# wendongbi/Bridged-GNN

Hardware: AMD Instinct MI355X
Metric: aggregated_edges_per_sec_ktgnn_fwd (higher is better)
Workload: dtype f32; 1 GPU; C4 synthetic bridged graph (local) N=1000000 E'=20991058, 2-layer KT-GNN eval fwd F=128 hidden=128 C=2; parallelism=single, execution=eager launches

## Files before the change

### bridged_gnn_amd/csrc/bgnn_aggregate.hip

```cpp
#include <cstdlib>
#include "bgnn_common.h"

namespace {

struct AggParams {
  const float* h_t2s;
  const float* h_s2t;
  int64_t ldh;
  const float* a_t2s;
  const float* a_s2t;
  const int32_t* rowptr;
  const int32_t* col;
  const uint8_t* mask;
  int64_t row_begin;
  int64_t row_end;
  int32_t D;
  float slope;
  float* out;
  int64_t ldo;
  float* alpha;
  const float* ep_scale;
  const float* ep_shift;
  int ep_relu;
  unsigned int* tile_queue;
// ... 857 lines not shown
  (void)ntiles; (void)grid;
  return forced > 0 ? forced : 4;
}

template <int HEADS, int EP, int U>
int launch_heads(const AggParams& p, hipStream_t st) {
  constexpr int RPB = 4 * (64 / (EP * HEADS));
  static const int cap = [] {
    int per_cu = 0, dev = 0;
    hipDeviceProp_t prop;
    if (hipGetDevice(&dev) != hipSuccess || hipGetDeviceProperties(&prop, dev) != hipSuccess) return 2048;
    if (hipOccupancyMaxActiveBlocksPerMultiprocessor(&per_cu, agg_heads_lanes_kernel<HEADS, EP, U>, 256, 0) != hipSuccess || per_cu < 1) return 2048;
    if (per_cu > 8) per_cu = 8;
    return per_cu * prop.multiProcessorCount / 8 * 8;
  }();
  const int64_t ntiles = (p.row_end - p.row_begin + p.n_vrows + RPB - 1) / RPB;
  int64_t grid = ntiles < cap ? (ntiles + 7) / 8 * 8 : cap;
  if (grid < 8) grid = 8;
  hipLaunchKernelGGL((agg_heads_lanes_kernel<HEADS, EP, U>), dim3((unsigned)grid), dim3(256), 0, st, p);
  BGNN_LAUNCH_CHECK();
  return 0;
}

template <int LF, int EP, int U>
int resident_blocks() {
  static const int nb = [] {
    int per_cu = 0, dev = 0;
    hipDeviceProp_t prop;
    if (hipGetDevice(&dev) != hipSuccess || hipGetDeviceProperties(&prop, dev) != hipSuccess) return 2048;
    if (hipOccupancyMaxActiveBlocksPerMultiprocessor(&per_cu, agg_kernel<LF, EP, U>, 256, 0) != hipSuccess || per_cu < 1)
      return 2048;
    if (per_cu > 8) per_cu = 8;
    return per_cu * prop.multiProcessorCount / 8 * 8;
  }();
  return nb;
}

template <int LF, int EP, int U>
int launch(const AggParams& p, hipStream_t st) {
  constexpr int RPB = 4 * (64 / (LF * EP));
  int64_t ntiles = ((p.row_end - p.row_begin) * p.heads + RPB - 1) / RPB;
  const int64_t cap = resident_blocks<LF, EP, U>();
  int64_t grid = ntiles < cap ? (ntiles + 7) / 8 * 8 : cap;
  if (grid < 8) grid = 8;
  AggParams q = p;
  q.tq_chunk = tq_chunk_for(ntiles, grid);
// ... 27 lines not shown
  hipLaunchKernelGGL((agg_wide_kernel<LF, U>), dim3((unsigned)grid), dim3(256), 0, st, q);
  BGNN_LAUNCH_CHECK();
  return 0;
}

static bool fast_plan(AggParams& p, int64_t table_rows) {
  static const bool on = [] { const char* e = getenv("BGNN_AGG_FAST"); return !(e && atoi(e) == 0); }();
  if (!on || table_rows <= 0) return false;
  if (p.heads != 1 || p.mode != 0 || p.n_vrows != 0 || p.hub_threshold != 0) return false;
  const int64_t lim24 = (int64_t)1 << 24, lim32 = ((int64_t)1 << 32) - 1;
  if (table_rows > lim24 || p.row_end > table_rows || p.ldh * 4 >= lim24 || p.ldo * 4 >= lim24) return false;
  const char* a = reinterpret_cast<const char*>(p.h_t2s);
  const char* b = reinterpret_cast<const char*>(p.h_s2t);
  const char* lo = a < b ? a : b;
  const int64_t span = (int64_t)((a < b ? b : a) - lo) + table_rows * p.ldh * 4;
  if (span > lim32 || p.row_end * p.ldo * 4 > lim32) return false;
  p.tbl_base = lo;
  p.tbl_bytes = (uint32_t)span;
  p.off_t2s = (uint32_t)(a - lo);
  p.off_s2t = (uint32_t)(b - lo);
  const int64_t lane_max = (span - table_rows * p.ldh * 4) + p.ldh * 4, dead = (((int64_t)1 << 32) - 16) - lane_max;
  p.dead_off = dead >= span ? (uint32_t)dead : 0u;
  return true;
}

template <int LF, bool ALPHA>
int launch_wide_fast(const AggParams& p, hipStream_t st) {
  constexpr int RPB = 4 * (64 / LF);
  static const int per_cu_max = [] {
    int per_cu = 0;
    if (hipOccupancyMaxActiveBlocksPerMultiprocessor(&per_cu, agg_wide_fast_kernel<LF, ALPHA>, 256, 0) != hipSuccess || per_cu < 1) return 0;
    if (per_cu > 8) per_cu = 8;
    const char* e = getenv("BGNN_AGG_BLOCKS_PER_CU");
    if (e && atoi(e) > 0 && atoi(e) < per_cu) per_cu = atoi(e);
    return per_cu;
  }();
  static const int n_cu = [] {
    int dev = 0;
    hipDeviceProp_t prop;
    if (hipGetDevice(&dev) != hipSuccess || hipGetDeviceProperties(&prop, dev) != hipSuccess) return 0;
    return prop.multiProcessorCount;
  }();
  static const bool forced = getenv("BGNN_AGG_BLOCKS_PER_CU") != nullptr;
  int per_cu = per_cu_max;
  if (p.gather_hint == 2 && !forced && per_cu > 3) per_cu = 3;
  const int64_t cap = (per_cu_max > 0 && n_cu > 0) ? (int64_t)per_cu * n_cu / 8 * 8 : 2048;
// ... 125 lines not shown
    p.state_ms[2 * (node * p.heads + h)] = m;
    p.state_ms[2 * (node * p.heads + h) + 1] = s;
  }
  if (p.ep_relu == 2) {
    float mx = r.x;
    if (p.D > 1) mx = fmaxf(mx, r.y);
    if (p.D > 2) mx = fmaxf(mx, r.z);
    if (p.D > 3) mx = fmaxf(mx, r.w);
    float se = expf(r.x - mx);
    if (p.D > 1) se += expf(r.y - mx);
    if (p.D > 2) se += expf(r.z - mx);
    if (p.D > 3) se += expf(r.w - mx);
    const float lse = logf(se);
    r.x = r.x - mx - lse;
    r.y = p.D > 1 ? r.y - mx - lse : 0.f;
    r.z = p.D > 2 ? r.z - mx - lse : 0.f;
    r.w = p.D > 3 ? r.w - mx - lse : 0.f;
  }
  *reinterpret_cast<float4*>(p.out + (node * p.heads + h) * p.ldo) = r;
}

static int dispatch_aggregate(const AggParams& p, hipStream_t st, int64_t table_rows = 0) {
  const int32_t D = p.D, heads = p.heads;
  if (heads == 3 && D <= 4 && p.ldh == 4 && p.ldo == 4) return launch_heads<3, 2, 4>(p, st);
  if (heads == 2 && D <= 4 && p.ldh == 4 && p.ldo == 4) return launch_heads<2, 2, 4>(p, st);
  const int nv = (D + 3) / 4;
  if (nv <= 1) return launch<1, 4, 4>(p, st);
  if (nv <= 2) return launch<2, 2, 4>(p, st);
  if (nv <= 4) return launch<4, 1, 8>(p, st);
  if (nv <= 8) return launch<8, 1, 4>(p, st);
  const bool wide_ok = p.slope >= 0.f && p.slope <= 1.f && (int64_t)heads * p.ldh * 4 < (int64_t)1 << 32;
  if (wide_ok) {
    AggParams q = p;
    if (fast_plan(q, table_rows)) {
      if (q.alpha != nullptr) {
        if (nv <= 16) return launch_wide_fast<16, true>(q, st);
        if (nv <= 32) return launch_wide_fast<32, true>(q, st);
        return launch_wide_fast<64, true>(q, st);
      }
      if (nv <= 16) return launch_wide_fast<16, false>(q, st);
      if (nv <= 32) return launch_wide_fast<32, false>(q, st);
      return launch_wide_fast<64, false>(q, st);
    }
    if (nv <= 16) return launch_wide<16, 4>(p, st);
    if (nv <= 32) return launch_wide<32, 4>(p, st);
    return launch_wide<64, 4>(p, st);
  }
// ... 14 lines not shown
                          const float* a_t2s, const float* a_s2t,
                          const int32_t* rowptr, const int32_t* col, const uint8_t* mask,
                          int64_t row_begin, int64_t row_end, int32_t D, float negative_slope,
                          float* out, int64_t ldo, float* alpha_opt,
                          const float* ep_scale_opt, const float* ep_shift_opt, int ep_relu,
                          float* state_ms_opt, int part, int64_t park_begin, int32_t heads,
                          double* colsum_opt, uint32_t* tile_queue_opt, int64_t table_rows, int32_t gather_hint, void* stream) {
  if (colsum_opt && heads != 1) return BGNN_E_SHAPE;
  if (part == 1 && (park_begin < row_begin || park_begin > row_end)) return BGNN_E_SHAPE;
  if (part < 0 || part > 3 || (part != 0 && (!state_ms_opt || alpha_opt))) return BGNN_E_NULL;
  if (part == 3 && !((heads == 3 || heads == 2) && D <= 4 && ldh == 4 && ldo == 4)) return BGNN_E_SHAPE;
  if (heads < 1 || heads > 8 || (heads > 1 && (alpha_opt || ep_scale_opt))) return BGNN_E_SHAPE;
  if (ep_relu < 0 || ep_relu > 2) return BGNN_E_SHAPE;
  if (ep_relu == 2 && !((heads == 3 || heads == 2) && D <= 4 && ldh == 4 && ldo == 4)) return BGNN_E_SHAPE;
  if (!h_t2s || !h_s2t || !a_t2s || !a_s2t || !rowptr || !col || !mask || !out) return BGNN_E_NULL;
  if (row_begin < 0 || row_end < row_begin || D <= 0 || D > 256 || ldh < D || ldo < D) return BGNN_E_SHAPE;
  if ((ldh & 3) || (ldo & 3) || !bgnn_aligned16(h_t2s) || !bgnn_aligned16(h_s2t) || !bgnn_aligned16(out))
    return BGNN_E_ALIGN;
  if ((ep_scale_opt == nullptr) != (ep_shift_opt == nullptr)) return BGNN_E_NULL;
  if (row_end == row_begin) return 0;
  AggParams p{h_t2s, h_s2t, ldh, a_t2s, a_s2t, rowptr, col, mask, row_begin, row_end, D, negative_slope,
              out, ldo, alpha_opt, ep_scale_opt, ep_shift_opt, ep_relu, tile_queue_opt, colsum_opt, heads, state_ms_opt, part,
              park_begin, 4};
  p.gather_hint = gather_hint;
  hipStream_t st = (hipStream_t)stream;
  if (tile_queue_opt) {
    hipError_t e = bgnn_zero_async(tile_queue_opt, 8 * sizeof(uint32_t), st);
    if (e != hipSuccess) return (int)e;
  }
  return dispatch_aggregate(p, st, table_rows);
}

extern "C" int bgnn_adaptedconv_aggregate_f32(const float* h_t2s, const float* h_s2t, int64_t ldh,
                                              const float* a_t2s, const float* a_s2t,
                                              const int32_t* rowptr, const int32_t* col, const uint8_t* mask,
                                              int64_t row_begin, int64_t row_end, int32_t D, float negative_slope,
                                              float* out, int64_t ldo, float* alpha_opt,
                                              const float* ep_scale_opt, const float* ep_shift_opt, int ep_relu,
                                              float* state_ms_opt, int part, int64_t park_begin, int32_t heads,
                                              double* colsum_opt, uint32_t* tile_queue_opt, void* stream) {
  return aggregate_impl(h_t2s, h_s2t, ldh, a_t2s, a_s2t, rowptr, col, mask, row_begin, row_end, D, negative_slope, out, ldo, alpha_opt,
                        ep_scale_opt, ep_shift_opt, ep_relu, state_ms_opt, part, park_begin, heads, colsum_opt, tile_queue_opt, 0, 0, stream);
}

extern "C" int bgnn_adaptedconv_aggregate_bounded_f32(const float* h_t2s, const float* h_s2t, int64_t ldh,
                                                      const float* a_t2s, const float* a_s2t,
                                                      const int32_t* rowptr, const int32_t* col, const uint8_t* mask,
                                                      int64_t row_begin, int64_t row_end, int32_t D, float negative_slope,
                                                      float* out, int64_t ldo, float* alpha_opt,
                                                      const float* ep_scale_opt, const float* ep_shift_opt, int ep_relu,
                                                      float* state_ms_opt, int part, int64_t park_begin, int32_t heads,
                                                      double* colsum_opt, uint32_t* tile_queue_opt, int64_t table_rows, int32_t gather_hint,
                                                      void* stream) {
  if (table_rows < row_end || gather_hint < 0 || gather_hint > 2) return BGNN_E_SHAPE;
  return aggregate_impl(h_t2s, h_s2t, ldh, a_t2s, a_s2t, rowptr, col, mask, row_begin, row_end, D, negative_slope, out, ldo, alpha_opt,
                        ep_scale_opt, ep_shift_opt, ep_relu, state_ms_opt, part, park_begin, heads, colsum_opt, tile_queue_opt, table_rows, gather_hint, stream);
}

extern "C" size_t bgnn_aggregate_hub_workspace_bytes(int64_t n_segments, int32_t heads, int64_t ldo) {
  const size_t nv = (size_t)(n_segments > 0 ? n_segments : 0), h = (size_t)(heads > 0 ? heads : 1);
  return bgnn_align_up(sizeof(float) * nv * h * (size_t)(ldo > 0 ? ldo : 0), 256) + bgnn_align_up(sizeof(float) * 2 * nv * h, 256) + 256;
}

extern "C" int bgnn_adaptedconv_aggregate_hub_f32(const float* h_t2s, const float* h_s2t, int64_t ldh,
                                                  const float* a_t2s, const float* a_s2t,
                                                  const int32_t* rowptr, const int32_t* col, const uint8_t* mask,
                                                  int64_t N, int32_t D, float negative_slope, float* out, int64_t ldo,
                                                  const float* ep_scale_opt, const float* ep_shift_opt, int ep_relu,
                                                  float* state_ms_opt, int32_t heads, double* colsum_opt,
                                                  uint32_t* tile_queue_opt, int32_t hub_threshold, const int32_t* hub_rows,
                                                  int64_t n_hubs, const int32_t* hub_seg_ptr, const int32_t* seg_bounds,
                                                  const int32_t* seg_node, int64_t n_segments, float* alpha_opt,
                                                  void* ws, size_t ws_bytes, void* stream) {
  if (!h_t2s || !h_s2t || !a_t2s || !a_s2t || !rowptr || !col || !mask || !out) return BGNN_E_NULL;
  if (alpha_opt && heads != 1) return BGNN_E_SHAPE;
  if (n_hubs > 0 && (!hub_rows || !hub_seg_ptr || !seg_bounds || !seg_node || !ws)) return BGNN_E_NULL;
  if (N < 0 || D <= 0 || D > 256 || ldh < D || ldo < D || (ldh & 3) || (ldo & 3) || hub_threshold < 2 || n_hubs < 0 || n_segments < n_hubs)
// ... 86 lines not shown
```

### bridged_gnn_amd/ktgnn.py

```python
import math
import os
import weakref

import torch
import torch.nn.functional as F
from torch import nn

from . import ops

__all__ = ["Linear", "AdaptedConv", "KTGNN_no_complement"]


def _plist(module):
    pl = module.__dict__.get("_bgnn_plist")
    if pl is None:
        pl = list(module.parameters())
        module.__dict__["_bgnn_plist"] = pl
    return pl


def _forget_plists(root):
    for m in root.modules():
        m.__dict__.pop("_bgnn_plist", None)

# ... 457 lines not shown

    def _versions(self):
        return tuple((p.data_ptr(), p._version) for p in _plist(self))

    def packed(self, din_pad, partner=None):
        key = (din_pad, self._versions(), partner._versions() if partner is not None else None)
        if getattr(self, "_pack_key", None) != key:
            heads = [self.head()] + ([partner.head()] if partner is not None else [])
            self._pack = ops.pack_transform_heads(heads, din_pad)
            self._pack_key = key
        return self._pack

    def transform(self, x, mask_u8, delta=None, sums=None, out=None, partner=None, tail_single=(0, 0), tile_need=None):
        xp = _pad_cols4(x)
        din_pad = xp.shape[1]
        if delta is None and sums is None:
            sums = ops.domain_sums(xp, mask_u8)
        res = ops.adaptedconv_transform(xp, mask_u8, delta, self.packed(din_pad, partner),
                                        out=out if (out is None or partner is not None) else [out],
                                        sums=sums if delta is None else None, tail_single=tail_single,
                                        tile_need=tile_need if (delta is None and partner is None) else None)
        return res if partner is not None else res[0]

    def aggregate(self, h_t2s, h_s2t, csr, mask_u8, n_dst=None, want_alpha=False, epilogue=None, colsum=None):
        a_t2s = self.a_f_t2s.weight.detach().reshape(-1).contiguous()
        a_s2t = self.a_f_s2t.weight.detach().reshape(-1).contiguous()
        sc, sh, relu = epilogue if epilogue is not None else (None, None, False)
        return ops.adaptedconv_aggregate(h_t2s, h_s2t, a_t2s, a_s2t, csr, mask_u8, self.out_channels,
                                         self.negative_slope, n_dst=n_dst, want_alpha=want_alpha,
                                         ep_scale=sc, ep_shift=sh, ep_relu=relu, colsum=colsum)

    def _transform_autograd(self, x, mask_u8, sums=None, mean_hook=None):
        return _TransformFn.apply(x, self.lin_s.weight, self.lin_s.bias, self.lin_t.weight, self.lin_t.bias,
                                  self.a_g_s2t.weight, self.a_g_t2s.weight, mask_u8, self, sums, mean_hook)

    def _forward_autograd(self, x, mask, mask_u8, csr, sums=None):
        D = self.out_channels
        if sums is not None and (x.requires_grad or sums.numel() != 2 * ops.pad4(x.shape[1]) + 2):
            sums = None
        h_t2s, h_s2t = _TransformFn.apply(x, self.lin_s.weight, self.lin_s.bias, self.lin_t.weight, self.lin_t.bias,
                                          self.a_g_s2t.weight, self.a_g_t2s.weight, mask_u8, self, sums)
        out = _AggregateFn.apply(h_t2s, h_s2t, self.a_f_t2s.weight.reshape(-1), self.a_f_s2t.weight.reshape(-1),
                                 csr, mask_u8, D, self.negative_slope)
        return out[:, :D]

    def _csr_for(self, edge_index, num_nodes):
        c = self._csr_cache
        if c is None or c[0]() is not edge_index or c[1] != edge_index._version or c[2] != num_nodes:
            csr = ops.build_dst_csr(edge_index, num_nodes, rewrite_self_loops=False)
            self._csr_cache = c = (weakref.ref(edge_index), edge_index._version, num_nodes, csr)
        return c[3]

    def forward(self, x, edge_index, edge_index1=None, edge_index2=None, central_mask=None, size=None,
                csr=None, delta=None, epilogue=None, return_alpha=False, colsum=None, sums=None):
        if isinstance(x, (tuple, list)):
            x_src, x_r = x
        else:
            x_src = x_r = x
        if not x_src.is_cuda:
            raise RuntimeError("AdaptedConv runs on MI355X only (CUDA/HIP tensors); there is no CPU path")
        if central_mask is None:
            raise ValueError("central_mask is required")
        x_src = x_src.float()
        N = x_src.shape[0]
        mask_u8 = _as_u8(central_mask).contiguous()
        if csr is None:
            csr = self._csr_for(edge_index, N)
        if torch.is_grad_enabled() and (x_src.requires_grad or any(p.requires_grad for p in _plist(self))):
            out = self._forward_autograd(x_src, central_mask.bool(), mask_u8, csr, sums=sums)
            if self.root_weight and x_r is not None:
                out = out + self.lin_r(x_r.float())
            if self.normalize:
                out = F.normalize(out, p=2.0, dim=-1)
            if epilogue is not None:
                sc, sh, relu = epilogue
                out = out * sc + sh
                out = F.relu(out) if relu else out
            return out
        if delta is None and sums is None:
            sums = ops.domain_sums(_pad_cols4(x_src), mask_u8)
        need = csr.tile_need(mask_u8) if (delta is None and csr.num_nodes == N and self.out_channels > 32 and _TILE_NEED) else None
        h_t2s, h_s2t = self.transform(x_src, mask_u8, delta=delta, sums=sums, tile_need=need)
        fuse = epilogue if not (self.root_weight or self.normalize) else None
        if colsum is not None and (fuse is None and epilogue is not None or self.root_weight or self.normalize):
            raise ValueError("colsum needs the fused epilogue path")
        res = self.aggregate(h_t2s, h_s2t, csr, mask_u8, want_alpha=return_alpha, epilogue=fuse, colsum=colsum)
        out, alpha = res if return_alpha else (res, None)
        out = out[:, : self.out_channels]
        if self.root_weight and x_r is not None:
            out = out + self.lin_r(x_r.float())
        if self.normalize:
            out = F.normalize(out, p=2.0, dim=-1)
        if epilogue is not None and fuse is None:
            sc, sh, relu = epilogue
            out = out * sc + sh
            out = F.relu(out) if relu else out
        return (out, alpha) if return_alpha else out

    def __repr__(self):
        return f"{self.__class__.__name__}({self.in_channels}, {self.out_channels})"


class KTGNN_no_complement(_PlistHooks, nn.Module):

    def __init__(self, num_features, num_classes=2, layer_num=2, hidden=64, root_weight=False, dim_share=300,
                 step=1, hidden_o=128, hidden_u=128, use_dist_loss=False, cached_edges=True, dropout=0.5,
                 use_bn=False, need_complement=False):
        super().__init__()
        if need_complement:
# ... 36 lines not shown
            n = central_mask.shape[0]
            edge_index = edge_index[:, edge_index[0] != edge_index[1]]
            loop = torch.arange(n, dtype=torch.int64, device=edge_index.device)
            edge_index = torch.cat([edge_index, torch.stack([loop, loop])], dim=1)
        m1 = central_mask[edge_index[1]]
        e1, e2 = edge_index[:, m1], edge_index[:, ~m1]
        return e1, e2, torch.cat((e1, e2), dim=-1)

    def _prepare(self, data):
        if self.cached_edges and self._csr is not None:
            return self._csr
        csr = ops.build_dst_csr(data.edge_index, data.central_mask.shape[0], rewrite_self_loops=True)
        if self.cached_edges:
            self._csr = csr
        return csr

    def _hidden(self, x, csr, central_mask, want_sums=False, arena=None):
        sums = None
        for ind, conv in enumerate(self.convs):
            sums_in, sums = sums, None
            if self.use_bn and not self.training and not (torch.is_grad_enabled() and any(p.requires_grad for p in _plist(conv))):
                sc, sh = bn_eval_affine(self.bns[ind])
                if arena is None:
                    arena = ops.ZeroArena(x.device, (len(self.convs) + 3) * (2 * ops.pad4(max(x.shape[1], conv.out_channels)) + 2))
                if sums_in is None and x.dtype == torch.float32 and x.stride(1) == 1 and x.shape[1] % 4 == 0:
                    sums_in = self._input_domain_sums(x, central_mask, arena)
                if not (conv.root_weight or conv.normalize):
                    sums = arena.take(2 * ops.pad4(conv.out_channels) + 2)
                x = conv(x, None, central_mask=central_mask, csr=csr, epilogue=(sc, sh, True), colsum=sums, sums=sums_in)
            else:
                if (ind == 0 and sums_in is None and torch.is_grad_enabled() and not x.requires_grad and x.dtype == torch.float32
                        and x.stride(1) == 1 and x.shape[1] % 4 == 0):
                    sums_in = self._input_domain_sums(x, central_mask, ops.ZeroArena(x.device, 2 * x.shape[1] + 2) if self._input_sums_miss(x, central_mask) else None)
                x = conv(x, None, central_mask=central_mask, csr=csr, sums=sums_in)
                if self.use_bn and self.training and torch.is_grad_enabled():
                    x = bn_relu_dropout_train(x, self.bns[ind], True, self.dropout)
                else:
                    if self.use_bn:
                        x = self.bns[ind](x)
                    x = F.relu(x)
                    x = F.dropout(x, p=self.dropout, training=self.training)
        self._arena = arena
        return (x, sums) if want_sums else x

    def _input_sums_miss(self, x, central_mask):
        if torch.cuda.is_current_stream_capturing() or not getattr(self, "cache_input_sums", True):
            return True
        c = getattr(self, "_xsum_cache", None)
        return not (c is not None and c[0]() is x and c[1] == x._version and c[2]() is central_mask and c[3] == central_mask._version)

    def _input_domain_sums(self, x, central_mask, arena):
        if torch.cuda.is_current_stream_capturing() or not getattr(self, "cache_input_sums", True):
# ... 16 lines not shown
        csr = self._prepare(data)
        x, sums_h = self._hidden(x, csr, central_mask, want_sums=True)
        x = x.contiguous()
        mask_u8 = _as_u8(central_mask).contiguous()
        stage = self._stage
        train = self.training and torch.is_grad_enabled()
        walk = stage.train_walk(opt_in=True) if (train and stage.plain and x.dtype == torch.float32) else None
        if walk is not None:
            sums_x = ops.domain_sums(_pad_cols4(x.detach()), mask_u8)
            tabs = stage.train_tables(x, mask_u8, sums_x, bn_relu_dropout_train)
            return (*stage.train_aggregate(walk, csr, mask_u8, tabs), None)
        if not stage.plain or torch.is_grad_enabled() or self.training:
            logits_base = self.clf_base(x, None, central_mask=central_mask, csr=csr)
            logits_target = self.clf_target(x, None, central_mask=central_mask, csr=csr)
            needs_grad = torch.is_grad_enabled() and (x.requires_grad or any(p.requires_grad for p in _plist(self.clf_transformer)))
            if train:
                l0, bn, _, l3 = self.clf_transformer
                xt = l3(bn_relu_dropout_train(l0(x), bn, True, 0.0))
            else:
                xt = self.clf_transformer(x) if (self.training or needs_grad) else stage.transformer_eval(x)
            logits_hat = self.clf_target(xt.contiguous(), None, central_mask=central_mask, csr=csr)
            return (F.log_softmax(logits_base, dim=1), F.log_softmax(logits_target, dim=1),
                    F.log_softmax(logits_hat, dim=1), None)
        t2s = torch.empty(x.shape[0], 3 * stage.ld, dtype=torch.float32, device=x.device)
        s2t = torch.empty_like(t2s)
        stage.eval_tables(x, mask_u8, sums_h, stage.views(t2s, s2t), self._arena)
        a_t2s, a_s2t = stage.attention()
        out3 = ops.adaptedconv_aggregate(t2s, s2t, a_t2s, a_s2t, csr, mask_u8, stage.C, stage.slope, heads=3,
                                         log_softmax=stage.fused_log_softmax)
        return (*stage.finish(out3), None)

    def graphed(self, data, warmup=2):
        if self.training:
            raise RuntimeError("graphed() captures the eval forward; call model.eval() first")
        with torch.no_grad():
            for _ in range(max(int(warmup), 1)):
                self.forward(data)
            torch.cuda.synchronize()
            g = torch.cuda.CUDAGraph()
            with torch.cuda.graph(g):
                out = self.forward(data)

        def replay():
            g.replay()
            return out
        replay.graph = g
        return replay

# ... 54 lines not shown
```

### bridged_gnn_amd/ops.py

```python
import os

import torch

from . import _lib as L

__all__ = ["DstCSR", "build_dst_csr", "domain_delta", "pack_transform_heads", "adaptedconv_transform", "adaptedconv_aggregate", "linear", "linear_supported", "linear_narrow_supported", "linear_narrow_transform", "narrow_transform_finish", "gram", "gram_supported", "rowdot", "transform_bwd_prep", "topk_edges_coalesced",
           "l2_normalize_rows", "cosine_topk", "mlp_pair_topk", "topk_edges", "coalesce", "gather_rows", "pad4",
           "sage_mean_aggregate", "sage_mean_aggregate_bwd", "rows_segment_add", "gcn_aggregate", "gcn_aggregate_bwd", "wide_heads_supported",
           "adaptedconv_aggregate_heads_wide", "adaptedconv_aggregate_heads_wide_bwd", "pair_csr", "pair_mlp_stats", "pair_mlp_loss",
           "pair_mlp_segsum", "pair_mlp_eval", "pair_mlp_count", "PAIR_MLP_WIDTH", "pair_cos_loss", "pair_cos_segsum", "pair_cos_count",
           "PAIR_COS_WIDTH"]


def pad4(n):
    return (int(n) + 3) // 4 * 4


HUB_THRESHOLD = 128
HUB_SEGMENT = 64


class DstCSR:

    def __init__(self, rowptr, col, eperm, num_edges, num_nodes):
# ... 403 lines not shown
            raise ValueError("adaptedconv_transform needs delta [Din] or the float64 domain sums [2*Din+2]")
        fn, first, name = lib.bgnn_adaptedconv_transform_sums_f32, sums, "bgnn_adaptedconv_transform_sums_f32"
    else:
        fn, first, name = lib.bgnn_adaptedconv_transform_f32, delta, "bgnn_adaptedconv_transform_f32"
    tail = (int(tail_single[0]), int(tail_single[1])) if delta is None else ()
    if delta is not None and tuple(tail_single) != (0, 0):
        raise ValueError("tail_single needs the sums form of the transform")
    if tile_need is not None:
        if delta is not None or tuple(tail_single) != (0, 0):
            raise ValueError("tile_need needs the sums form of the transform and no tail_single")
        if tile_need.dtype != torch.int32 or tile_need.numel() != (N + 31) // 32:
            raise ValueError("tile_need: one int32 per 32-row tile")
        fn, name, tail = lib.bgnn_adaptedconv_transform_need_f32, "bgnn_adaptedconv_transform_need_f32", (L.ptr(tile_need),)
    rc = fn(L.ptr(x), N, Din, x.stride(0), L.ptr(mask_u8), L.ptr(first), H, D, L.ptr(Wp), L.ptr(bp), L.ptr(gates), L.ptr(gconst),
            L.ptr_rows(out[0][1]), L.ptr_rows(out[0][0]), L.ptr_rows(o1[1]), L.ptr_rows(o1[0]), ldh, row_stride, *tail,
            L.ptr(small), L.stream())
    L.check(rc, name)
    return out


_P2_STATIC = os.environ.get("BGNN_P2_STATIC", "1") != "0"


def _tile_queue(dev):
    return torch.empty(8, dtype=torch.int32, device=dev)


def heads_log_softmax_supported(heads, D):
    return heads in (2, 3) and D <= 4


def _hub_shape_ok(D, ldh, ldo, heads, slope):
    if heads in (2, 3) and D <= 4 and ldh == 4 and ldo == 4:
        return True
    return heads == 1 and D > 32 and 0.0 <= slope <= 1.0


def adaptedconv_aggregate(h_t2s, h_s2t, a_t2s, a_s2t, csr, mask_u8, D, negative_slope=0.1, n_dst=None,
                          want_alpha=False, ep_scale=None, ep_shift=None, ep_relu=False, out=None,
                          row_begin=0, row_end=None, state_ms=None, part=0, heads=1, colsum=None, log_softmax=False,
                          park_begin=None):
    lib = L.lib()
    n_dst = csr.num_nodes if n_dst is None else int(n_dst)
    row_end = n_dst if row_end is None else int(row_end)
    ldh = h_t2s.stride(0) // heads
    ldo = pad4(D)
    dev = h_t2s.device
    if out is None:
        out = torch.empty(n_dst, heads * ldo, dtype=torch.float32, device=dev)
    assert h_t2s.stride(0) == h_s2t.stride(0) and h_t2s.stride(0) % heads == 0 and out.stride(0) % heads == 0
    alpha = torch.empty(csr.num_edges, dtype=torch.float32, device=dev) if want_alpha else None
    tq = _tile_queue(dev) if heads == 1 else None
    if row_end <= int(row_begin):
        return (out, alpha) if want_alpha else out
    if ((not want_alpha or heads == 1) and part in (0, 3) and int(row_begin) == 0 and row_end == csr.num_nodes == n_dst and h_t2s.shape[0] == n_dst
            and (ep_scale is None or heads == 1) and _hub_shape_ok(D, ldh, out.stride(0) // heads, heads, negative_slope)
            and os.environ.get("BGNN_HUB_ROWS", "1") != "0"):
        hubs = csr.hub_tables()
        if hubs is not None:
            hub_rows, seg_ptr, seg_bounds, seg_node = hubs
            nseg = int(seg_node.numel())
            wsb = lib.bgnn_aggregate_hub_workspace_bytes(nseg, heads, out.stride(0) // heads)
            ws = torch.empty(wsb, dtype=torch.uint8, device=dev)
            rc = lib.bgnn_adaptedconv_aggregate_hub_f32(
                L.ptr_rows(h_t2s), L.ptr_rows(h_s2t), ldh, L.ptr(a_t2s), L.ptr(a_s2t), L.ptr(csr.rowptr), L.ptr(csr.col),
                L.ptr(mask_u8), n_dst, D, float(negative_slope), L.ptr_rows(out), out.stride(0) // heads,
                L.ptr(ep_scale), L.ptr(ep_shift), 2 if log_softmax else (1 if ep_relu else 0),
                L.ptr(state_ms) if part == 3 else None, int(heads), L.ptr(colsum),
                L.ptr(tq), HUB_THRESHOLD, L.ptr(hub_rows), int(hub_rows.numel()),
                L.ptr(seg_ptr), L.ptr(seg_bounds), L.ptr(seg_node), nseg, L.ptr(alpha), L.ptr(ws), wsb, L.stream())
            L.check(rc, "bgnn_adaptedconv_aggregate_hub_f32")
            return (out, alpha) if want_alpha else out
    rc = lib.bgnn_adaptedconv_aggregate_bounded_f32(
        L.ptr_rows(h_t2s), L.ptr_rows(h_s2t), ldh, L.ptr(a_t2s), L.ptr(a_s2t), L.ptr(csr.rowptr), L.ptr(csr.col),
        L.ptr(mask_u8), int(row_begin), row_end, D, float(negative_slope), L.ptr_rows(out), out.stride(0) // heads, L.ptr(alpha),
        L.ptr(ep_scale), L.ptr(ep_shift), 2 if log_softmax else (1 if ep_relu else 0), L.ptr(state_ms), int(part),
        int(row_begin) if park_begin is None else int(park_begin), int(heads), L.ptr(colsum),
        L.ptr(tq) if not (part == 2 and _P2_STATIC) else None, min(int(h_t2s.shape[0]), int(h_s2t.shape[0])),
        csr.gather_hint() if (heads == 1 and D > 32 and part == 0) else 0, L.stream())
    L.check(rc, "bgnn_adaptedconv_aggregate_bounded_f32")
    return (out, alpha) if want_alpha else out


def adaptedconv_aggregate_bwd(h_t2s, h_s2t, a_t2s, a_s2t, csr, mask_u8, D, out, alpha, grad_out, negative_slope=0.1):
    lib = L.lib()
    dev = h_t2s.device
    da_t2s = torch.zeros(D, dtype=torch.float32, device=dev)
    da_s2t = torch.zeros(D, dtype=torch.float32, device=dev)
    grad_out = grad_out.contiguous()
    if D <= 128 and grad_out.stride(0) % 4 == 0 and grad_out.data_ptr() % 16 == 0 and h_t2s.shape[0] == csr.num_nodes:
        t_rowptr, t_eid, t_dst = csr.transposed()
        dh_t2s, dh_s2t = torch.empty_like(h_t2s), torch.empty_like(h_s2t)
        narrow = D <= 4 and h_t2s.stride(0) == 4 and out.stride(0) == 4 and grad_out.stride(0) == 4
        dh_, sh_ = (csr.hub_tables(), csr.transposed_hub_tables()) if (not narrow and os.environ.get("BGNN_HUB_ROWS", "1") != "0") else (None, None)
        if dh_ is not None or sh_ is not None:
            none4 = (None, None, None, None)
            d_rows, d_ptr, d_bounds, d_node = dh_ if dh_ is not None else none4
            s_rows, s_ptr, s_bounds, s_node = sh_ if sh_ is not None else none4
            nd = 0 if dh_ is None else int(d_node.numel())
            ns = 0 if sh_ is None else int(s_node.numel())
            wsb = lib.bgnn_aggregate_bwd_pull_hub_workspace_bytes(csr.num_nodes, csr.num_edges, h_t2s.stride(0), nd, ns)
            ws = torch.empty(wsb, dtype=torch.uint8, device=dev)
# ... 667 lines not shown
```

### include/bgnn.h

```cpp
#ifndef BGNN_H_
#define BGNN_H_
#include <stddef.h>
#include <stdint.h>

#ifdef __cplusplus
extern "C" {
#endif

#define BGNN_VERSION 113
#define BGNN_E_NULL (-1)
#define BGNN_E_SHAPE (-2)
#define BGNN_E_WORKSPACE (-3)
#define BGNN_E_ALIGN (-4)
#define BGNN_E_RANGE (-5)

int bgnn_version(void);
const char* bgnn_error_string(int code);
const char* bgnn_source_hash(void);

size_t bgnn_csr_workspace_bytes(int64_t N, int64_t E);
int bgnn_build_dst_csr(const int64_t* edge_index, int64_t E, int64_t N, int rewrite_self_loops,
                       int32_t* rowptr, int32_t* col, int32_t* eperm_opt, int64_t* E_out_dev,
                       void* ws, size_t ws_bytes, void* stream);

// ... 56 lines not shown
                                        const uint8_t* mask, const double* sums,
                                        int32_t n_heads, int32_t D, const float* Wp, const float* bias_p,
                                        const float* gates, const float* gate_const_opt,
                                        float* h_s2t_0, float* h_t2s_0, float* h_s2t_1, float* h_t2s_1,
                                        int64_t ldh, int64_t row_stride, int64_t n_tail_t2s, int64_t n_tail_s2t,
                                        float* small_ws, void* stream);
int bgnn_adaptedconv_transform_need_f32(const float* x, int64_t N, int32_t Din, int64_t ldx,
                                        const uint8_t* mask, const double* sums,
                                        int32_t n_heads, int32_t D, const float* Wp, const float* bias_p,
                                        const float* gates, const float* gate_const_opt,
                                        float* h_s2t_0, float* h_t2s_0, float* h_s2t_1, float* h_t2s_1,
                                        int64_t ldh, int64_t row_stride, const int32_t* tile_need_opt,
                                        float* small_ws, void* stream);

int bgnn_adaptedconv_aggregate_f32(const float* h_t2s, const float* h_s2t, int64_t ldh,
                                   const float* a_t2s, const float* a_s2t,
                                   const int32_t* rowptr, const int32_t* col, const uint8_t* mask,
                                   int64_t row_begin, int64_t row_end, int32_t D, float negative_slope,
                                   float* out, int64_t ldo, float* alpha_opt,
                                   const float* ep_scale_opt, const float* ep_shift_opt, int ep_relu,
                                   float* state_ms_opt, int part, int64_t park_begin, int32_t heads, double* colsum_opt,
                                   uint32_t* tile_queue_opt, void* stream);

int bgnn_adaptedconv_aggregate_bounded_f32(const float* h_t2s, const float* h_s2t, int64_t ldh,
                                           const float* a_t2s, const float* a_s2t,
                                           const int32_t* rowptr, const int32_t* col, const uint8_t* mask,
                                           int64_t row_begin, int64_t row_end, int32_t D, float negative_slope,
                                           float* out, int64_t ldo, float* alpha_opt,
                                           const float* ep_scale_opt, const float* ep_shift_opt, int ep_relu,
                                           float* state_ms_opt, int part, int64_t park_begin, int32_t heads, double* colsum_opt,
                                           uint32_t* tile_queue_opt, int64_t table_rows, int32_t gather_hint, void* stream);

size_t bgnn_aggregate_hub_workspace_bytes(int64_t n_segments, int32_t heads, int64_t ldo);
int bgnn_adaptedconv_aggregate_hub_f32(const float* h_t2s, const float* h_s2t, int64_t ldh,
                                       const float* a_t2s, const float* a_s2t,
                                       const int32_t* rowptr, const int32_t* col, const uint8_t* mask,
                                       int64_t N, int32_t D, float negative_slope, float* out, int64_t ldo,
                                       const float* ep_scale_opt, const float* ep_shift_opt, int ep_relu,
                                       float* state_ms_opt, int32_t heads, double* colsum_opt,
                                       uint32_t* tile_queue_opt, int32_t hub_threshold, const int32_t* hub_rows,
                                       int64_t n_hubs, const int32_t* hub_seg_ptr, const int32_t* seg_bounds,
                                       const int32_t* seg_node, int64_t n_segments, float* alpha_opt,
                                       void* ws, size_t ws_bytes, void* stream);

int bgnn_adaptedconv_aggregate_bwd_f32(const float* h_t2s, const float* h_s2t, int64_t ldh,
                                       const float* a_t2s, const float* a_s2t,
// ... 200 lines not shown
```

Baseline: 50.56 billion edges/s.

## Add opt-in fast 3-head aggregate kernel and pre-zeroed tile queues from arena

Adds a specialized 3-head aggregation kernel that uses buffer-resource gathers, inline-asm prefetch of column ids and per-D vector widths. It is gated behind the BGNN_HEADS_FAST environment variable, so it is off by default. Separately, the eval forward now takes pre-zeroed tile-queue slots from the zero arena and flags them, which skips the per-call async memset and the per-call queue allocation. The two head tables are also allocated in one tensor so they sit adjacent for the 32-bit buffer span. The default-on part mainly removes a small launch and memset per layer.

```diff
diff --git a/bridged_gnn_amd/csrc/bgnn_aggregate.hip b/bridged_gnn_amd/csrc/bgnn_aggregate.hip
--- a/bridged_gnn_amd/csrc/bgnn_aggregate.hip
+++ b/bridged_gnn_amd/csrc/bgnn_aggregate.hip
@@ -903,6 +903,178 @@
   return 0;
 }
 
+template <int NC> struct HeadsVec { typedef float type __attribute__((ext_vector_type(NC))); };
+template <> struct HeadsVec<1> { typedef float type; };
+typedef unsigned int u32x2_t __attribute__((ext_vector_type(2)));
+
+template <int NC>
+__device__ __forceinline__ typename HeadsVec<NC>::type heads_gather(__amdgpu_buffer_rsrc_t r, uint32_t off) {
+  typedef typename HeadsVec<NC>::type V;
+  if constexpr (NC == 1) return __builtin_bit_cast(V, __builtin_amdgcn_raw_buffer_load_b32(r, off, 0, 0));
+  else if constexpr (NC == 2) return __builtin_bit_cast(V, __builtin_amdgcn_raw_buffer_load_b64(r, off, 0, 0));
+  else return __builtin_bit_cast(V, __builtin_amdgcn_raw_buffer_load_b128(r, off, 0, 0));
+}
+template <int NC>
+__device__ __forceinline__ float hv_get(const typename HeadsVec<NC>::type& v, int c) {
+  if constexpr (NC == 1) return v; else return v[c];
+}
+template <int NC>
+__device__ __forceinline__ void hv_set(typename HeadsVec<NC>::type& v, int c, float x) {
+  if constexpr (NC == 1) v = x; else v[c] = x;
+}
+
+template <int NC>
+__global__ __launch_bounds__(256) void agg_heads_fast_kernel(AggParams p) {
+  static_assert(NC == 1 || NC == 2 || NC == 4, "live floats of a 16-byte head slot");
+  constexpr int HEADS = 3, EP = 2, U = 4, GL = EP * HEADS, GPW = 64 / GL, RPB = 4 * GPW;
+  typedef typename HeadsVec<NC>::type V;
+  const int lane = threadIdx.x & 63, wave = threadIdx.x >> 6;
+  const int g = lane / GL, lg = lane - g * GL;
+  const int sub = lg / HEADS, h = lg - sub * HEADS;
+  const bool lane_on = g < GPW;
+  const int32_t row0 = (int32_t)p.row_begin, row1 = (int32_t)p.row_end;
+  const int32_t ntiles = (row1 - row0 + RPB - 1) / RPB;
+  const int32_t xcd = blockIdx.x % 8, nslots = ((int32_t)gridDim.x + 7 - xcd) / 8;
+  const int32_t per = (ntiles + 7) / 8, seg_len = (per + bgnn::XCD_NSEG - 1) / bgnn::XCD_NSEG;
+  const int32_t pos_end = xcd * per + bgnn::XCD_NSEG * seg_len;
+  constexpr uint32_t rs = HEADS * 16u;
+  const __amdgpu_buffer_rsrc_t rt = __builtin_amdgcn_make_buffer_rsrc(const_cast<char*>(p.tbl_base), (short)0, (int)p.tbl_bytes, 0x00020000);
+  V aS, aT, sl;
+#pragma unroll
+  for (int c = 0; c < NC; ++c) {
+    hv_set<NC>(aS, c, c < p.D ? p.a_t2s[h * p.D + c] : 0.f);
+    hv_set<NC>(aT, c, c < p.D ? p.a_s2t[h * p.D + c] : 0.f);
+    hv_set<NC>(sl, c, p.slope);
+  }
+  for (int32_t pos = xcd * per + (int32_t)(blockIdx.x / 8); pos < pos_end; pos += nslots) {
+    const int32_t j = pos - xcd * per, sg = j / seg_len;
+    const int32_t tile = (sg * 8 + xcd) * seg_len + (j - sg * seg_len);
+    if (tile >= ntiles) continue;
+    const int32_t i = row0 + tile * RPB + wave * GPW + g;
+    const bool rvalid = lane_on && i < row1;
+    const int32_t ic = rvalid ? i : row0;
+    const bool dom_s = p.mask[ic] != 0;
+    const int32_t beg = rvalid ? p.rowptr[ic] : 0;
+    const int32_t end = rvalid ? p.rowptr[ic + 1] : 0;
+    const int32_t wbeg = __builtin_amdgcn_readlane(beg, 0);
+    const int32_t* __restrict__ wcol = p.col + wbeg;
+    const int32_t rend = rvalid ? end - wbeg : 0;
+    const int32_t rlast = max(rend - 1, 0);
+    int32_t er = (rvalid ? beg - wbeg : 0) + sub;
+    const uint32_t lbase = (dom_s ? p.off_t2s : p.off_s2t) + (uint32_t)h * 16u;
+    const uint32_t dead = lbase + p.dead_off;
+    const V a = dom_s ? aS : aT;
+    V hi = heads_gather<NC>(rt, lbase + __umul24((uint32_t)ic, rs));
+    const int32_t niter = (end - beg + EP * U - 1) / (EP * U);
+    int32_t nw = __builtin_amdgcn_readlane(niter, 0);
+#pragma unroll
+    for (int k = 1; k < GPW; ++k) nw = max(nw, __builtin_amdgcn_readlane(niter, k * GL));
+
+    V acc;
+#pragma unroll
+    for (int c = 0; c < NC; ++c) hv_set<NC>(acc, c, 0.f);
+    float m = -INFINITY, s = 0.f;
+    uint32_t id[U] = {0u, 0u, 0u, 0u};
+    auto load_ids = [&](int32_t e) {
+      const uint32_t o0 = (uint32_t)min(e, rlast) * 4u, o1 = (uint32_t)min(e + EP, rlast) * 4u;
+      const uint32_t o2 = (uint32_t)min(e + 2 * EP, rlast) * 4u, o3 = (uint32_t)min(e + 3 * EP, rlast) * 4u;
+      __builtin_amdgcn_sched_barrier(0);
+      asm volatile("global_load_dword %0, %4, %8\n\tglobal_load_dword %1, %5, %8\n\t"
+                   "global_load_dword %2, %6, %8\n\tglobal_load_dword %3, %7, %8"
+                   : "=&v"(id[0]), "=&v"(id[1]), "=&v"(id[2]), "=&v"(id[3])
+                   : "v"(o0), "v"(o1), "v"(o2), "v"(o3), "s"(wcol) : "memory");
+      __builtin_amdgcn_sched_barrier(0);
+    };
+    auto take_ids = [&]() {
+      __builtin_amdgcn_sched_barrier(0);
+      asm volatile("s_waitcnt vmcnt(0)" : "+v"(id[0]), "+v"(id[1]), "+v"(id[2]), "+v"(id[3]), "+v"(m), "+v"(s), "+v"(acc) : : "memory");
+    };
+    if (nw > 0) {
+      load_ids(er);
+      take_ids();
+    }
+    for (int32_t it = 0; it < nw; ++it) {
+      bool ok[U];
+      V v[U];
+#pragma unroll
+      for (int u = 0; u < U; ++u) ok[u] = er + u * EP < rend;
+#pragma unroll
+      for (int u = 0; u < U; ++u) {
+        uint32_t o = __umul24(id[u], rs) + lbase;
+        asm("" : "+v"(o));
+        v[u] = heads_gather<NC>(rt, ok[u] ? o : dead);
+      }
+      asm volatile("" : "+v"(hi) : : "memory");
+      __builtin_amdgcn_sched_barrier(0);
+      er += EP * U;
+      load_ids(er);
+      float lg_[U], cm = -INFINITY;
+#pragma unroll
+      for (int u = 0; u < U; ++u) {
+        V z = v[u] + hi;
+        z = __builtin_elementwise_max(z, z * sl);
+        float t = hv_get<NC>(a, 0) * hv_get<NC>(z, 0);
+#pragma unroll
+        for (int c = 1; c < NC; ++c) t = fmaf(hv_get<NC>(a, c), hv_get<NC>(z, c), t);
+        lg_[u] = ok[u] ? t : -INFINITY;
+        cm = fmaxf(cm, lg_[u]);
+      }
+      const float mn = fmaxf(m, cm);
+      const float sc = (m == mn) ? 1.f : __expf(m - mn);
+      acc = acc * sc;
+#pragma unroll
+      for (int u = 0; u < U; ++u) {
+        const float pe = (lg_[u] == -INFINITY) ? 0.f : __expf(lg_[u] - mn);
+        s = u == 0 ? fmaf(s, sc, pe) : s + pe;
+        if constexpr (NC == 1) acc = fmaf(pe, v[u], acc);
+        else { V pv; for (int c = 0; c < NC; ++c) pv[c] = pe; acc = __builtin_elementwise_fma(pv, v[u], acc); }
+      }
+      m = mn;
+      take_ids();
+    }
+#pragma unroll
+    for (int off = 1; off < EP; off <<= 1) {
+      const int src = (sub ^ off) * HEADS + h + g * GL;
+      const int from = lane_on ? src : lane;
+      const float m2 = __shfl(m, from), s2 = __shfl(s, from);
+      float b[NC];
+#pragma unroll
+      for (int c = 0; c < NC; ++c) b[c] = __shfl(hv_get<NC>(acc, c), from);
+      const float mn = fmaxf(m, m2);
+      const float c1 = (m == mn) ? 1.f : __expf(m - mn), c2 = (m2 == mn) ? 1.f : __expf(m2 - mn);
+      s = fmaf(s, c1, s2 * c2);
+#pragma unroll
+      for (int c = 0; c < NC; ++c) hv_set<NC>(acc, c, fmaf(hv_get<NC>(acc, c), c1, b[c] * c2));
+      m = mn;
+    }
+    if (rvalid && sub == 0) {
+#pragma clang fp contract(off)
+      const int64_t oh = (int64_t)i * HEADS + h;
+      const float inv = 1.f / (s + 1e-16f);
+      float r[4] = {0.f, 0.f, 0.f, 0.f};
+#pragma unroll
+      for (int c = 0; c < NC; ++c) r[c] = hv_get<NC>(acc, c) * inv;
+      if (p.mode == 3) {
+        p.state_ms[2 * oh] = m;
+        p.state_ms[2 * oh + 1] = s;
+      }
+      if (p.ep_relu == 2) {
+        float mx = r[0];
+#pragma unroll
+        for (int c = 1; c < NC; ++c) if (p.D > c) mx = fmaxf(mx, r[c]);
+        float se = expf(r[0] - mx);
+#pragma unroll
+        for (int c = 1; c < NC; ++c) if (p.D > c) se += expf(r[c] - mx);
+        const float lse = logf(se);
+        r[0] = r[0] - mx - lse;
+#pragma unroll
+        for (int c = 1; c < NC; ++c) r[c] = p.D > c ? r[c] - mx - lse : 0.f;
+      }
+      *reinterpret_cast<float4*>(p.out + oh * 4) = make_float4(r[0], r[1], r[2], r[3]);
+    }
+  }
+}
+
 template <int LF, int EP, int U>
 int resident_blocks() {
   static const int nb = [] {
@@ -976,6 +1148,51 @@
   const int64_t lane_max = (span - table_rows * p.ldh * 4) + p.ldh * 4, dead = (((int64_t)1 << 32) - 16) - lane_max;
   p.dead_off = dead >= span ? (uint32_t)dead : 0u;
   return true;
+}
+
+static int heads_fast_switch() {
+  static const bool on = [] { const char* e = getenv("BGNN_AGG_FAST"); return !(e && atoi(e) == 0); }();
+  const char* hf = getenv("BGNN_HEADS_FAST");
+  return (on && hf) ? atoi(hf) : 0;
+}
+static bool heads_fast_plan(AggParams& p, int64_t table_rows) {
+  if (table_rows <= 0) return false;
+  if (p.heads != 3 || p.D > 4 || p.ldh != 4 || p.ldo != 4 || (p.mode != 0 && p.mode != 3) || p.n_vrows != 0 || p.hub_threshold != 0) return false;
+  if (p.alpha != nullptr || p.ep_scale != nullptr || !(p.slope >= 0.f && p.slope <= 1.f)) return false;
+  const int64_t lim24 = (int64_t)1 << 24, lim32 = ((int64_t)1 << 32) - 1, rs = 3 * 16;
+  if (table_rows > lim24 || p.row_end > table_rows || p.row_begin < 0) return false;
+  const char* a = reinterpret_cast<const char*>(p.h_t2s);
+  const char* b = reinterpret_cast<const char*>(p.h_s2t);
+  const char* lo = a < b ? a : b;
+  const int64_t upper = (int64_t)((a < b ? b : a) - lo), span = upper + table_rows * rs;
+  if (span > lim32) return false;
+  const int64_t dead = (((int64_t)1 << 32) - 16) - (upper + rs);
+  if (dead < span) return false;
+  p.tbl_base = lo;
+  p.tbl_bytes = (uint32_t)span;
+  p.off_t2s = (uint32_t)(a - lo);
+  p.off_s2t = (uint32_t)(b - lo);
+  p.dead_off = (uint32_t)dead;
+  return true;
+}
+
+template <int NC>
+int launch_heads_fast(const AggParams& p, hipStream_t st) {
+  constexpr int RPB = 4 * (64 / 6);
+  static const int cap = [] {
+    int per_cu = 0, dev = 0;
+    hipDeviceProp_t prop;
+    if (hipGetDevice(&dev) != hipSuccess || hipGetDeviceProperties(&prop, dev) != hipSuccess) return 2048;
+    if (hipOccupancyMaxActiveBlocksPerMultiprocessor(&per_cu, agg_heads_fast_kernel<NC>, 256, 0) != hipSuccess || per_cu < 1) return 2048;
+    if (per_cu > 8) per_cu = 8;
+    return per_cu * prop.multiProcessorCount / 8 * 8;
+  }();
+  const int64_t ntiles = (p.row_end - p.row_begin + RPB - 1) / RPB;
+  int64_t grid = ntiles < cap ? (ntiles + 7) / 8 * 8 : cap;
+  if (grid < 8) grid = 8;
+  hipLaunchKernelGGL((agg_heads_fast_kernel<NC>), dim3((unsigned)grid), dim3(256), 0, st, p);
+  BGNN_LAUNCH_CHECK();
+  return 0;
 }
 
 template <int LF, bool ALPHA>
@@ -1147,7 +1364,17 @@
 
 static int dispatch_aggregate(const AggParams& p, hipStream_t st, int64_t table_rows = 0) {
   const int32_t D = p.D, heads = p.heads;
-  if (heads == 3 && D <= 4 && p.ldh == 4 && p.ldo == 4) return launch_heads<3, 2, 4>(p, st);
+  if (heads == 3 && D <= 4 && p.ldh == 4 && p.ldo == 4) {
+    AggParams q = p;
+    const int sw = heads_fast_switch();
+    if (sw != 0 && heads_fast_plan(q, table_rows)) {
+      if (D == 1) return launch_heads_fast<1>(q, st);
+      if (D == 2) return launch_heads_fast<2>(q, st);
+      return launch_heads_fast<4>(q, st);
+    }
+    if (sw == 2) return BGNN_E_SHAPE;
+    return launch_heads<3, 2, 4>(p, st);
+  }
   if (heads == 2 && D <= 4 && p.ldh == 4 && p.ldo == 4) return launch_heads<2, 2, 4>(p, st);
   const int nv = (D + 3) / 4;
   if (nv <= 1) return launch<1, 4, 4>(p, st);
@@ -1208,9 +1435,9 @@
   AggParams p{h_t2s, h_s2t, ldh, a_t2s, a_s2t, rowptr, col, mask, row_begin, row_end, D, negative_slope,
               out, ldo, alpha_opt, ep_scale_opt, ep_shift_opt, ep_relu, tile_queue_opt, colsum_opt, heads, state_ms_opt, part,
               park_begin, 4};
-  p.gather_hint = gather_hint;
+  p.gather_hint = gather_hint & ~BGNN_TILE_QUEUE_ZEROED;
   hipStream_t st = (hipStream_t)stream;
-  if (tile_queue_opt) {
+  if (tile_queue_opt && !(gather_hint & BGNN_TILE_QUEUE_ZEROED)) {
     hipError_t e = bgnn_zero_async(tile_queue_opt, 8 * sizeof(uint32_t), st);
     if (e != hipSuccess) return (int)e;
   }
@@ -1238,7 +1465,10 @@
                                                       float* state_ms_opt, int part, int64_t park_begin, int32_t heads,
                                                       double* colsum_opt, uint32_t* tile_queue_opt, int64_t table_rows, int32_t gather_hint,
                                                       void* stream) {
+  const bool queue_zeroed = gather_hint >= 0 && (gather_hint & BGNN_TILE_QUEUE_ZEROED) != 0;
+  if (queue_zeroed) gather_hint -= BGNN_TILE_QUEUE_ZEROED;
   if (table_rows < row_end || gather_hint < 0 || gather_hint > 2) return BGNN_E_SHAPE;
+  if (queue_zeroed && tile_queue_opt) gather_hint |= BGNN_TILE_QUEUE_ZEROED;
   return aggregate_impl(h_t2s, h_s2t, ldh, a_t2s, a_s2t, rowptr, col, mask, row_begin, row_end, D, negative_slope, out, ldo, alpha_opt,
                         ep_scale_opt, ep_shift_opt, ep_relu, state_ms_opt, part, park_begin, heads, colsum_opt, tile_queue_opt, table_rows, gather_hint, stream);
 }
diff --git a/bridged_gnn_amd/ktgnn.py b/bridged_gnn_amd/ktgnn.py
--- a/bridged_gnn_amd/ktgnn.py
+++ b/bridged_gnn_amd/ktgnn.py
@@ -503,13 +503,13 @@
                                         tile_need=tile_need if (delta is None and partner is None) else None)
         return res if partner is not None else res[0]
 
-    def aggregate(self, h_t2s, h_s2t, csr, mask_u8, n_dst=None, want_alpha=False, epilogue=None, colsum=None):
+    def aggregate(self, h_t2s, h_s2t, csr, mask_u8, n_dst=None, want_alpha=False, epilogue=None, colsum=None, tile_queue=None):
         a_t2s = self.a_f_t2s.weight.detach().reshape(-1).contiguous()
         a_s2t = self.a_f_s2t.weight.detach().reshape(-1).contiguous()
         sc, sh, relu = epilogue if epilogue is not None else (None, None, False)
         return ops.adaptedconv_aggregate(h_t2s, h_s2t, a_t2s, a_s2t, csr, mask_u8, self.out_channels,
                                          self.negative_slope, n_dst=n_dst, want_alpha=want_alpha,
-                                         ep_scale=sc, ep_shift=sh, ep_relu=relu, colsum=colsum)
+                                         ep_scale=sc, ep_shift=sh, ep_relu=relu, colsum=colsum, tile_queue=tile_queue)
 
     def _transform_autograd(self, x, mask_u8, sums=None, mean_hook=None):
         return _TransformFn.apply(x, self.lin_s.weight, self.lin_s.bias, self.lin_t.weight, self.lin_t.bias,
@@ -533,7 +533,7 @@
         return c[3]
 
     def forward(self, x, edge_index, edge_index1=None, edge_index2=None, central_mask=None, size=None,
-                csr=None, delta=None, epilogue=None, return_alpha=False, colsum=None, sums=None):
+                csr=None, delta=None, epilogue=None, return_alpha=False, colsum=None, sums=None, tile_queue=None):
         if isinstance(x, (tuple, list)):
             x_src, x_r = x
         else:
@@ -565,7 +565,7 @@
         fuse = epilogue if not (self.root_weight or self.normalize) else None
         if colsum is not None and (fuse is None and epilogue is not None or self.root_weight or self.normalize):
             raise ValueError("colsum needs the fused epilogue path")
-        res = self.aggregate(h_t2s, h_s2t, csr, mask_u8, want_alpha=return_alpha, epilogue=fuse, colsum=colsum)
+        res = self.aggregate(h_t2s, h_s2t, csr, mask_u8, want_alpha=return_alpha, epilogue=fuse, colsum=colsum, tile_queue=tile_queue)
         out, alpha = res if return_alpha else (res, None)
         out = out[:, : self.out_channels]
         if self.root_weight and x_r is not None:
@@ -648,12 +648,13 @@
             if self.use_bn and not self.training and not (torch.is_grad_enabled() and any(p.requires_grad for p in _plist(conv))):
                 sc, sh = bn_eval_affine(self.bns[ind])
                 if arena is None:
-                    arena = ops.ZeroArena(x.device, (len(self.convs) + 3) * (2 * ops.pad4(max(x.shape[1], conv.out_channels)) + 2))
+                    arena = ops.ZeroArena(x.device, (len(self.convs) + 3) * (2 * ops.pad4(max(x.shape[1], conv.out_channels)) + 2) + 4 * len(self.convs))
                 if sums_in is None and x.dtype == torch.float32 and x.stride(1) == 1 and x.shape[1] % 4 == 0:
                     sums_in = self._input_domain_sums(x, central_mask, arena)
                 if not (conv.root_weight or conv.normalize):
                     sums = arena.take(2 * ops.pad4(conv.out_channels) + 2)
-                x = conv(x, None, central_mask=central_mask, csr=csr, epilogue=(sc, sh, True), colsum=sums, sums=sums_in)
+                x = conv(x, None, central_mask=central_mask, csr=csr, epilogue=(sc, sh, True), colsum=sums, sums=sums_in,
+                         tile_queue=arena.take(4).view(torch.int32))
             else:
                 if (ind == 0 and sums_in is None and torch.is_grad_enabled() and not x.requires_grad and x.dtype == torch.float32
                         and x.stride(1) == 1 and x.shape[1] % 4 == 0):
@@ -716,8 +717,7 @@
             logits_hat = self.clf_target(xt.contiguous(), None, central_mask=central_mask, csr=csr)
             return (F.log_softmax(logits_base, dim=1), F.log_softmax(logits_target, dim=1),
                     F.log_softmax(logits_hat, dim=1), None)
-        t2s = torch.empty(x.shape[0], 3 * stage.ld, dtype=torch.float32, device=x.device)
-        s2t = torch.empty_like(t2s)
+        t2s, s2t = torch.empty(2, x.shape[0], 3 * stage.ld, dtype=torch.float32, device=x.device).unbind(0)
         stage.eval_tables(x, mask_u8, sums_h, stage.views(t2s, s2t), self._arena)
         a_t2s, a_s2t = stage.attention()
         out3 = ops.adaptedconv_aggregate(t2s, s2t, a_t2s, a_s2t, csr, mask_u8, stage.C, stage.slope, heads=3,
diff --git a/bridged_gnn_amd/ops.py b/bridged_gnn_amd/ops.py
--- a/bridged_gnn_amd/ops.py
+++ b/bridged_gnn_amd/ops.py
@@ -449,6 +449,9 @@
 _P2_STATIC = os.environ.get("BGNN_P2_STATIC", "1") != "0"
 
 
+_TILE_QUEUE_ZEROED = 4
+
+
 def _tile_queue(dev):
     return torch.empty(8, dtype=torch.int32, device=dev)
 
@@ -466,7 +469,7 @@
 def adaptedconv_aggregate(h_t2s, h_s2t, a_t2s, a_s2t, csr, mask_u8, D, negative_slope=0.1, n_dst=None,
                           want_alpha=False, ep_scale=None, ep_shift=None, ep_relu=False, out=None,
                           row_begin=0, row_end=None, state_ms=None, part=0, heads=1, colsum=None, log_softmax=False,
-                          park_begin=None):
+                          park_begin=None, tile_queue=None):
     lib = L.lib()
     n_dst = csr.num_nodes if n_dst is None else int(n_dst)
     row_end = n_dst if row_end is None else int(row_end)
@@ -477,7 +480,10 @@
         out = torch.empty(n_dst, heads * ldo, dtype=torch.float32, device=dev)
     assert h_t2s.stride(0) == h_s2t.stride(0) and h_t2s.stride(0) % heads == 0 and out.stride(0) % heads == 0
     alpha = torch.empty(csr.num_edges, dtype=torch.float32, device=dev) if want_alpha else None
-    tq = _tile_queue(dev) if heads == 1 else None
+    own_tq = tile_queue is not None and heads == 1
+    if own_tq:
+        assert tile_queue.dtype == torch.int32 and tile_queue.numel() == 8 and tile_queue.is_contiguous()
+    tq = (tile_queue if own_tq else _tile_queue(dev)) if heads == 1 else None
     if row_end <= int(row_begin):
         return (out, alpha) if want_alpha else out
     if ((not want_alpha or heads == 1) and part in (0, 3) and int(row_begin) == 0 and row_end == csr.num_nodes == n_dst and h_t2s.shape[0] == n_dst
@@ -504,7 +510,7 @@
         L.ptr(ep_scale), L.ptr(ep_shift), 2 if log_softmax else (1 if ep_relu else 0), L.ptr(state_ms), int(part),
         int(row_begin) if park_begin is None else int(park_begin), int(heads), L.ptr(colsum),
         L.ptr(tq) if not (part == 2 and _P2_STATIC) else None, min(int(h_t2s.shape[0]), int(h_s2t.shape[0])),
-        csr.gather_hint() if (heads == 1 and D > 32 and part == 0) else 0, L.stream())
+        (csr.gather_hint() if (heads == 1 and D > 32 and part == 0) else 0) + (_TILE_QUEUE_ZEROED if own_tq else 0), L.stream())
     L.check(rc, "bgnn_adaptedconv_aggregate_bounded_f32")
     return (out, alpha) if want_alpha else out
 
diff --git a/include/bgnn.h b/include/bgnn.h
--- a/include/bgnn.h
+++ b/include/bgnn.h
@@ -102,6 +102,7 @@
                                    float* state_ms_opt, int part, int64_t park_begin, int32_t heads, double* colsum_opt,
                                    uint32_t* tile_queue_opt, void* stream);
 
+#define BGNN_TILE_QUEUE_ZEROED 4
 int bgnn_adaptedconv_aggregate_bounded_f32(const float* h_t2s, const float* h_s2t, int64_t ldh,
                                            const float* a_t2s, const float* a_s2t,
                                            const int32_t* rowptr, const int32_t* col, const uint8_t* mask,
```

Result: no change. 50.55 billion edges/s (-0.0%).
